# sparsemat/sprs

Hardware: AMD Instinct MI355X
Metric: CSR SpMV GFLOP/s (higher is better)
Workload: dtype f64; 1 GPU; R-MAT 10M x 10M, ~32 nnz/row (Graph500 a,b,c,d=.57,.19,.19,.05; seed 1); rows=10000000, cols=10000000, nnz=321592231, index_bytes=8, indptr_bytes=8, partition=single GPU, first_spmv_plan=nnz tiles

## Files before the change

sprs_amd/csrc/common.hpp:

```cpp
#pragma once

#include <hip/hip_runtime.h>
#include <cstdint>
#include <cstdio>
#include <memory>
#include <mutex>
#include <string>
#include <unordered_map>
#include <vector>

#include "../../include/sprs_hip.h"

struct sprs_hip_spgemm_plan;
struct sprs_hip_dist;

namespace sprs_hip {

void set_error(int32_t status, const char *fmt, ...) __attribute__((format(printf, 2, 3)));
int32_t fail_hip(hipError_t e, const char *what);
void clear_error();

#define SPRS_TRY_HIP(expr)                                              \
    do {                                                                \
        hipError_t e__ = (expr);                                        \
// ... 20 lines not shown
#define SPRS_HIP_OPTIONS(X)                                                                                                     \
    X(spmv_kernel, 0, 0, 2, 0)                                               \
    X(spmv_xcs, 0, 0, 2, 0)                                         \
    X(spmv_xcs_split, 32, 2, INT64_MAX, 0)                              \
    X(spmv_xcs_idx32, 1, 0, 1, 0)                                 \
    X(spmv_sort_tiles, 0, 0, 1, 0)               \
    X(spmv_relabel, 0, 0, 2, 0)                      \
    X(spmv_tile, 0, 0, 4096, 0)                                                 \
    X(spmv_lds_pad, 0, 0, 100000, 0)                  \
    X(spmv_xmask, -1, INT64_MIN, INT64_MAX, 1)       \
    X(spmv_plan_defer, 1, 0, 1, 0)       \
    X(spmv_band, 0, 0, 2, 0)                      \
    X(spmv_band_hot, 0, 0, 384, 0)                                                              \
    X(spmv_band_tile, 0, 0, 16384, 0)    \
    X(spmv_f32_band_tile, 0, 0, 32768, 0)  \
    X(spmv_band_phases, 0, 0, 8, 0)                        \
    X(spmv_band_split, 0, 0, INT64_MAX, 0)         \
    X(spmv_band_rounds, 0, 0, 64, 0)     \
    X(spmv_band_debug, 0, 0, 255, 1)     \
    X(spmv_band_tail, 0, 0, 2, 0)        \
    X(spmv_band_balance, 0, 0, 2, 0)     \
    X(spmv_band_xcd, 0, 0, 2, 0)         \
    X(spmv_band_pack, 0, 0, 2, 0)        \
    X(spmv_band_share, 0, 0, 1ll << 30, 0)  \
    X(spmv_band_hot_run, 0, 0, 4096, 0)  \
    X(spmv_band_cold_tiles, 0, 0, 64, 0)                  \
    X(spmv_band_overlap, 0, 0, 2, 0)         \
    X(spmv_band_split_permute, 0, 0, 2, 0)  \
    X(spmm_long_row, -1, -1, INT64_MAX, 0)  \
    X(spmm_stream, 1, 0, 1, 0)           \
    X(spgemm_micro, 0, 0, 2, 0)          \
    X(spgemm_task_order, 0, 0, 2, 0)      \
    X(spgemm_xcd_chunk, 0, -1, 0, 0)                \
    X(spgemm_bucket, 1, 0, 1, 0)                                   \
    X(spgemm_prof, 0, 0, 1, 1)                             \
    X(spgemm_tokens, 1, 1, 4, 0)                              \
    X(spgemm_keep_bits, 1, 0, 1, 0)      \
    X(spgemm_lane_order, 0, 0, 2, 0)     \
    X(spgemm_overlap, 0, 0, 1, 0)                                \
    X(spgemm_midwin_sym, 14, 14, 16, 0)                         \
    X(spgemm_mid_keep, 8, 4, 8, 0)       \
    X(spgemm_mid_keep_sym, 8, 8, 16, 0)  \
    X(spgemm_midwin, 15, 14, 15, 0)      \
    X(spgemm_mid, 65536, 0, 1ll << 31, 0)    \
    X(spgemm_ordered, 1, 0, 1, 0)        \
    X(spmm_relayout, 0, 0, 2, 0)         \
// ... 531 lines not shown
```

sprs_amd/csrc/spmv_band.hip:

```cpp
#include "spmv_band_kernels.hpp"

#include <algorithm>
#include <cstdlib>
#include <vector>

namespace sprs_hip {

namespace {

constexpr int MAX_HOT = 384;
constexpr int MAX_PHASES = 8;
constexpr int MAX_PIECES = MAX_HOT + 8 * MAX_PHASES + 1;

__global__ __launch_bounds__(256) void bp_inverse_kernel(const uint32_t *__restrict__ perm, uint64_t cols, uint32_t hot_labels,
                                                         uint32_t *__restrict__ inv_hot) {
    const uint64_t j = (uint64_t)blockIdx.x * blockDim.x + threadIdx.x;
    if (j >= cols) return;
    const uint32_t l = perm[j];
    if (l < hot_labels) inv_hot[l] = (uint32_t)j;
}

struct SliceMap {
    uint32_t nh, phases, xt_log2;
    uint64_t hot_labels;
    uint64_t phase_width;
};

__device__ __forceinline__ uint32_t piece_of_label(const SliceMap &m, uint64_t label) {
    if (label < m.hot_labels) return (uint32_t)(label >> m.xt_log2);
    uint64_t ph = (label - m.hot_labels) / m.phase_width;
    if (ph >= m.phases) ph = m.phases - 1;
    return m.nh + (uint32_t)ph * 8u + x_slice(label);
}

template <typename PTR>
__global__ void bp_classify_kernel(const PTR *__restrict__ indptr, uint64_t rows, uint64_t split,
                                   uint64_t *__restrict__ short_flag, uint64_t *__restrict__ short_len,
                                   uint64_t *__restrict__ long_flag) {
    const uint64_t r = (uint64_t)blockIdx.x * blockDim.x + threadIdx.x;
    if (r >= rows) return;
    const uint64_t len = (uint64_t)indptr[r + 1] - (uint64_t)indptr[r];
    const bool is_long = len >= split;
    short_flag[r] = (!is_long && len) ? 1 : 0;
    short_len[r] = is_long ? 0 : len;
    long_flag[r] = is_long ? 1 : 0;
}

struct ShortBuckets {
    const uint64_t *bucket0;
    uint64_t Rp, R;
};

__device__ __forceinline__ uint64_t short_place(const ShortBuckets &sb, uint64_t d) {
    if (!sb.bucket0) return d;
    const uint64_t k = d / sb.Rp;
    return k * sb.R + (d - sb.bucket0[k]);
}

__global__ void bp_bucket_starts_kernel(const uint64_t *__restrict__ short_ptr, uint64_t rows, uint64_t Rp, uint64_t nb,
                                        uint64_t *__restrict__ bucket0) {
    const uint64_t k = (uint64_t)blockIdx.x * blockDim.x + threadIdx.x;
    if (k >= nb) return;
    const uint64_t target = k * Rp;
    uint64_t lo = 0, hi = rows;
    while (lo < hi) {
        const uint64_t mid = (lo + hi) >> 1;
        if (short_ptr[mid] < target) lo = mid + 1;
        else hi = mid;
// ... 339 lines not shown
        if (fork) (void)hipEventDestroy(fork);
        if (join) (void)hipEventDestroy(join);
        if (aux) (void)hipStreamDestroy(aux);
    }
};

struct BandPlan {
    uint32_t nh = 0, phases = 1, npieces = 0;
    uint32_t xt_log2 = 14;
    uint32_t vbytes = 8;
    uint32_t n_long = 0, n_short_rows = 0;
    uint64_t cols = 0, cols_pad = 0;
    uint32_t *perm = nullptr, *long_rows = nullptr;
    uint32_t *inv_hot = nullptr;
    uint32_t nref = 0;
    uint32_t hot_labels = 0;
    void *vals_hot = nullptr, *vals_cold = nullptr;
    uint16_t *cid_hot = nullptr;
    unsigned char *packed_hot = nullptr;
    TileWord *hot_tw = nullptr;
    uint32_t hot_wgs_packed = 0;
    uint32_t *cid_cold = nullptr;
    uint32_t *rowidx_all = nullptr, *tile_row_all = nullptr;
    Seg *segs = nullptr;
    HotSeg *hsegs = nullptr;
    HotSeg *wg_first = nullptr;
    uint32_t *wg_seg = nullptr;
    uint32_t nranges = 0, nsegs = 0, hot_wgs = 0, cold_tiles = 4, hot_run = 4;
    void *spills_y = nullptr;
    void *rspills = nullptr;
    uint32_t *rsp_off = nullptr;
    uint32_t nspills = 0, nspills_y = 0;
    bool small = false;
    ColdGroup *groups = nullptr;
    unsigned long long *wmask = nullptr;
    uint32_t *wbase = nullptr;
    uint32_t np_pad = 0;
    uint64_t total_pairs = 0;
    uint32_t ngroups = 0, cold_blocks = 0, short_first_block = 0;
    bool has_short_group = false;
    std::vector<BandPiece> host_pieces;
    std::vector<uint64_t> pair_off;
    std::unordered_map<void *, BandScratch> scratch;
    uint64_t bytes = 0;
    DevBuf perm_block;
    std::vector<DevBuf> blocks;
// ... 197 lines not shown

    const uint64_t hot_entries = hot_tiles * WT;
    DevBuf vals_hot_blk, cid_hot_blk;
    SPRS_TRY_HIP(vals_hot_blk.alloc((hot_entries + WT) * VB));
    SPRS_TRY_HIP(cid_hot_blk.alloc((hot_entries + WT) * 2));
    bp->vals_hot = vals_hot_blk.p;
    bp->cid_hot = cid_hot_blk.as<uint16_t>();
    SPRS_TRY_HIP(hipMemsetAsync(bp->vals_hot, 0, (hot_entries + WT) * VB, stream));
    SPRS_TRY_HIP(hipMemsetAsync(bp->cid_hot, 0, (hot_entries + WT) * 2, stream));
    SPRS_TRY_HIP(alloc_block(bp->blocks, bp->vals_cold, (cold_ent + WT) * VB));
    SPRS_TRY_HIP(alloc_block(bp->blocks, bp->cid_cold, (cold_ent + WT) * 4));
    SPRS_TRY_HIP(hipMemsetAsync(bp->vals_cold, 0, (cold_ent + WT) * VB, stream));
    SPRS_TRY_HIP(hipMemsetD32Async((hipDeviceptr_t)bp->cid_cold, (int)(uint32_t)cols, cold_ent + WT, stream));
    DevBuf ptr_all;
    SPRS_TRY_HIP(ptr_all.alloc((ptr_off + n_short_rows + 2) * 4));
    SPRS_TRY_HIP(alloc_block(bp->blocks, bp->rowidx_all, (row_off + n_short_rows + 1) * 4));
    SPRS_TRY_HIP(alloc_block(bp->blocks, bp->tile_row_all, (tile_off + 1) * 4));
    bp->bytes = (cold_ent + WT) * (4 + VB) + (row_off + n_short_rows + tile_off) * 4 + cols * 4 + n_long * 4 +
                ((uint64_t)bp->nref + 4) * 4;
    hipLaunchKernelGGL((bp_fill_short_kernel<IDX, PTR, T>), dim3((unsigned)((rows + 256) / 256)), dim3(256), 0, stream, ip, ix,
                       (const T *)a->data, rows, short_pos.u64(), short_ptr.u64(), long_pos.u64(), bp->perm, (uint32_t *)nullptr,
                       (uint32_t *)s_ptr_t.p, bp->cid_cold, (T *)bp->vals_cold, bp->long_rows, split, 1, sbk, nnz_short_padded, n_long);
    SPRS_TRY_HIP(hipGetLastError());
    SPRS_TRY_HIP(hipMemcpyAsync((uint32_t *)ptr_all.p + ptr_off, s_ptr_t.p, (n_short_rows + 1) * 4, hipMemcpyDeviceToDevice, stream));
    if (n_short_rows)
        SPRS_TRY_HIP(hipMemcpyAsync(bp->rowidx_all + row_off, s_rowidx_t.p, n_short_rows * 4, hipMemcpyDeviceToDevice, stream));

    SPRS_TRY_HIP(pb_d.alloc(NP * sizeof(PieceBuild)));
    SPRS_TRY_HIP(hipMemcpyAsync(pb_d.p, pb.data(), NP * sizeof(PieceBuild), hipMemcpyHostToDevice, stream));
    hipLaunchKernelGGL((bp_scatter_kernel<IDX, PTR, T>), dim3((unsigned)wblocks), dim3(256), 0, stream, ip, ix, (const T *)a->data,
                       bp->long_rows, n_long, bp->perm, map, NP, pos.u64(), (const PieceBuild *)pb_d.p, (T *)bp->vals_hot,
                       bp->cid_hot, (T *)bp->vals_cold, bp->cid_cold);
    SPRS_TRY_HIP(hipGetLastError());
    hipLaunchKernelGGL(bp_rows_kernel, dim3((unsigned)((flat + 255) / 256)), dim3(256), 0, stream, cnt.u64(), pos.u64(),
                       pair.u64(), n_long, NP, (const PieceBuild *)pb_d.p, (uint32_t *)ptr_all.p, bp->rowidx_all);
    SPRS_TRY_HIP(hipGetLastError());

    {
        const uint64_t nwb = (n_long + WAVE - 1) / WAVE;
        bp->total_pairs = row_off;
        bp->np_pad = (NP + (uint32_t)RU - 1u) / (uint32_t)RU * (uint32_t)RU;
        const uint64_t slots = nwb * bp->np_pad;
        SPRS_TRY_HIP(alloc_block(bp->blocks, bp->wmask, (slots + WAVE) * 8));
        SPRS_TRY_HIP(alloc_block(bp->blocks, bp->wbase, (slots + WAVE) * 4));
        SPRS_TRY_HIP(hipMemsetAsync(bp->wmask, 0, (slots + WAVE) * 8, stream));
        SPRS_TRY_HIP(hipMemsetAsync(bp->wbase, 0, (slots + WAVE) * 4, stream));
// ... 318 lines not shown
    return dispatch_widths(a->idx_bytes, a->iptr_bytes, [&](auto i, auto p) {
        return band_build_t<typename decltype(i)::type, typename decltype(p)::type>(a, stream, out);
    });
}

int32_t band_prepare_stream(sprs_hip_csmat_f32 *a, BandPlan *bp, hipStream_t stream) {
    std::lock_guard<std::recursive_mutex> lock(a->mu);
    BandScratch *sc = nullptr;
    return band_scratch(bp, stream, &sc);
}

uint64_t band_plan_bytes(const BandPlan *bp) { return bp ? bp->bytes : 0; }

namespace {
template <typename T>
struct BandK;
template <>
struct BandK<double> {
    using Cold = ColdArgs;
    using Reduce = ReduceArgs;
    template <bool ACC, bool TOY>
    static auto cold() { return &band_cold_kernel<ACC, TOY>; }
    template <bool ACC>
    static auto reduce() { return &band_reduce_kernel<ACC>; }
    template <bool ACC>
    static auto tail() { return &band_tail_kernel<ACC>; }
    static auto permute() { return &band_permute_kernel; }
};
template <>
struct BandK<float> {
    using Cold = ColdArgsT<float>;
    using Reduce = ReduceArgsT<float>;
    template <bool ACC, bool TOY>
    static auto cold() { return &band_cold_kernel_f32<ACC, TOY>; }
    template <bool ACC>
    static auto reduce() { return &band_reduce_kernel_f32<ACC>; }
    template <bool ACC>
    static auto tail() { return &band_tail_kernel_f32<ACC>; }
    static auto permute() { return &band_permute_kernel_f32; }
};

template <typename H>
int32_t band_spmv_t(H *a, BandPlan *bp, const typename H::value_type *x, typename H::value_type *y, bool acc, hipStream_t stream) {
    using T = typename H::value_type;
    using K = BandK<T>;
    constexpr bool F32 = sizeof(T) == 4;
    BandScratch *sc = nullptr;
    {
        std::lock_guard<std::recursive_mutex> lock(a->mu);
        SPRS_TRY(band_scratch(bp, stream, &sc));
    }
    const bool overlap = options().spmv_band_overlap != 2 && bp->hot_wgs && bp->cold_blocks && (!bp->small || options().spmv_band_overlap == 1);
    const bool split_permute = overlap && options().spmv_band_split_permute != 2 && bp->hot_labels;
    const bool early_reduce = overlap && options().spmv_band_tail != 2;
    hipStream_t cstream = overlap ? sc->aux : stream;
    auto launch_carry_y = [&](hipStream_t st) -> int32_t {
        const uint32_t n = bp->nspills_y;
        if (!n) return SPRS_HIP_OK;
        hipLaunchKernelGGL((band_carry_kernel<true, T>), dim3((n + 255) / 256), dim3(256), 0, st, (const Spill *)bp->spills_y, n, (const T *)sc->carry,
                           (T *)sc->partial, y);
        SPRS_TRY_HIP(hipGetLastError());
        return SPRS_HIP_OK;
    };
    const uint32_t cut = bp->has_short_group ? bp->short_first_block : bp->cold_blocks;
    const bool fused_tail = !overlap && bp->small && options().spmv_band_tail != 2 && bp->cold_blocks > cut;
    auto launch_hot = [&]() -> int32_t {
        if (!bp->hot_wgs) return SPRS_HIP_OK;
        const uint32_t lds = F32 ? hot_lds_bytes_f32(bp->xt_log2) : hot_lds_bytes(bp->xt_log2);
#ifndef SPRS_HIP_EMU
        {
            static std::mutex mu;
            static std::unordered_map<int, bool> done;
            std::lock_guard<std::mutex> lock(mu);
            if constexpr (F32) {
                if (!done[a->device]) {
                    SPRS_TRY_HIP(hipFuncSetAttribute((const void *)band_hot_kernel_f32<13, 0>, hipFuncAttributeMaxDynamicSharedMemorySize, (int)hot_lds_bytes_f32(13)));
                    SPRS_TRY_HIP(hipFuncSetAttribute((const void *)band_hot_kernel_f32<14, 0>, hipFuncAttributeMaxDynamicSharedMemorySize, (int)hot_lds_bytes_f32(14)));
                    SPRS_TRY_HIP(hipFuncSetAttribute((const void *)band_hot_kernel_f32<15, 0>, hipFuncAttributeMaxDynamicSharedMemorySize, (int)hot_lds_bytes_f32(15)));
                    done[a->device] = true;
                }
            } else if (!done[a->device]) {
                const void *k13[] = {(const void *)band_hot_kernel<13, 0>, (const void *)band_hot_kernel<13, 1>, (const void *)band_hot_kernel<13, 2>};
                const void *k14[] = {(const void *)band_hot_kernel<14, 0>, (const void *)band_hot_kernel<14, 1>, (const void *)band_hot_kernel<14, 2>};
                for (const void *k : k13) SPRS_TRY_HIP(hipFuncSetAttribute(k, hipFuncAttributeMaxDynamicSharedMemorySize, (int)hot_lds_bytes(13)));
                for (const void *k : k14) SPRS_TRY_HIP(hipFuncSetAttribute(k, hipFuncAttributeMaxDynamicSharedMemorySize, (int)hot_lds_bytes(14)));
                done[a->device] = true;
            }
        }
// ... 49 lines not shown
                t1 = std::max(t1, t[3 * b + 2]);
            }
            std::vector<double> st, xw, du, en;
            for (uint32_t b = 0; b < bp->hot_wgs; ++b) {
                st.push_back((t[3 * b] - t0) * 0.01);
                xw.push_back((t[3 * b + 1] - t[3 * b]) * 0.01);
                du.push_back((t[3 * b + 2] - t[3 * b]) * 0.01);
                en.push_back((t[3 * b + 2] - t0) * 0.01);
            }
            auto q = [](std::vector<double> v, double f) {
                std::sort(v.begin(), v.end());
                return v[(size_t)(f * (v.size() - 1))];
            };
            fprintf(stderr, "[hot_prof] %u workgroups, span %.1f us | start min/med/p90/max %.1f %.1f %.1f %.1f | first x tile after %.1f %.1f %.1f %.1f | "
                            "duration %.1f %.1f %.1f %.1f | end %.1f %.1f %.1f %.1f\n", bp->hot_wgs, (t1 - t0) * 0.01,
                    q(st, 0), q(st, .5), q(st, .9), q(st, 1), q(xw, 0), q(xw, .5), q(xw, .9), q(xw, 1), q(du, 0), q(du, .5), q(du, .9), q(du, 1),
                    q(en, 0), q(en, .5), q(en, .9), q(en, 1));
        }
        return SPRS_HIP_OK;
    };
    auto cold_args = [&](uint32_t b0) {
        typename K::Cold ca;
        static_cast<ColdArgsT<T> &>(ca) = ColdArgsT<T>{sc->pieces, bp->groups, bp->ngroups, (const T *)bp->vals_cold, bp->cid_cold, (const T *)sc->xp, y, (T *)sc->carry,
                                                       b0, bp->cold_tiles, 0u, BandPiece()};
        return ca;
    };
    auto launch_gather = [&](uint32_t b0, uint32_t nb) -> int32_t {
        if (!nb) return SPRS_HIP_OK;
        const typename K::Cold ca = cold_args(b0);
        if (b0 < cut) hipLaunchKernelGGL((K::template cold<false, false>()), dim3(nb), dim3(CNT), 0, cstream, ca);
        else if (acc) hipLaunchKernelGGL((K::template cold<true, true>()), dim3(nb), dim3(CNT), 0, cstream, ca);
        else hipLaunchKernelGGL((K::template cold<false, true>()), dim3(nb), dim3(CNT), 0, cstream, ca);
        SPRS_TRY_HIP(hipGetLastError());
        return SPRS_HIP_OK;
    };

    const bool by_gather = (uint64_t)bp->nref * 3 <= bp->cols;
    auto launch_xp = [&](uint32_t l0, uint32_t l1, bool clear_y, hipStream_t st, bool hot_only = false) -> int32_t {
        if (!by_gather && !hot_only) {
            const uint64_t span = clear_y ? std::max<uint64_t>(bp->cols, a->rows) : bp->cols;
            hipLaunchKernelGGL((K::permute()), dim3((unsigned)((span + 1023) / 1024)), dim3(256), 0, st, x, (const uint32_t *)bp->perm, bp->cols,
                               (T *)sc->xp, clear_y ? y : (T *)nullptr, a->rows, l0, (uint32_t)bp->cols_pad);
            SPRS_TRY_HIP(hipGetLastError());
            return SPRS_HIP_OK;
        }
        const uint64_t n4 = std::max<uint64_t>(l1 > l0 ? ((uint64_t)(l1 - l0) + 3) / 4 : 0, clear_y ? (a->rows + 3) / 4 : 0);
        if (!n4) return SPRS_HIP_OK;
        if (clear_y)
            hipLaunchKernelGGL((band_gather_kernel<true, T>), dim3((unsigned)((n4 + 255) / 256)), dim3(256), 0, st, x, (const uint32_t *)bp->inv_hot, l0,
                               l1 > l0 ? l1 : l0, (T *)sc->xp, y, a->rows);
        else
            hipLaunchKernelGGL((band_gather_kernel<false, T>), dim3((unsigned)((n4 + 255) / 256)), dim3(256), 0, st, x, (const uint32_t *)bp->inv_hot, l0,
                               l1 > l0 ? l1 : l0, (T *)sc->xp, (T *)nullptr, a->rows);
        SPRS_TRY_HIP(hipGetLastError());
        return SPRS_HIP_OK;
    };
    const uint32_t hot_end = bp->hot_labels < bp->nref ? bp->hot_labels : bp->nref;
    if (split_permute) SPRS_TRY(launch_xp(0u, hot_end, false, stream, true));
    else SPRS_TRY(launch_xp(0u, bp->nref, !acc, stream));
    if (overlap) {
        SPRS_TRY_HIP(hipEventRecord(sc->fork, stream));
        SPRS_TRY(launch_hot());
        SPRS_TRY_HIP(hipStreamWaitEvent(sc->aux, sc->fork, 0));
    }
    if (split_permute) SPRS_TRY(launch_xp(hot_end, bp->nref, !acc, cstream));
    SPRS_TRY(launch_gather(0, cut));
    if (early_reduce) SPRS_TRY_HIP(hipEventRecord(sc->cold_done, sc->aux));
    if (!fused_tail) SPRS_TRY(launch_gather(cut, bp->cold_blocks - cut));
    if (early_reduce) SPRS_TRY(launch_carry_y(sc->aux));
    if (overlap) SPRS_TRY_HIP(hipEventRecord(sc->join, sc->aux));
    else SPRS_TRY(launch_hot());
    if (overlap) SPRS_TRY_HIP(hipStreamWaitEvent(stream, early_reduce ? sc->cold_done : sc->join, 0));
    if (!early_reduce && !fused_tail) SPRS_TRY(launch_carry_y(stream));
    const uint32_t nwb = (bp->n_long + WAVE - 1) / WAVE;
    const uint32_t per_xcd = (nwb + 7) / 8;
    const dim3 rg(((per_xcd + 3) / 4) * 8), rb(256);
    typename K::Reduce ra;
    static_cast<ReduceArgsT<T> &>(ra) = ReduceArgsT<T>{(const T *)sc->partial, bp->wmask, bp->wbase, bp->long_rows, (const RSpill *)bp->rspills,
                                                       bp->nspills ? bp->rsp_off : nullptr, (const T *)sc->carry, y, bp->n_long, bp->np_pad, nwb};
    if (fused_tail) {
        typename K::Cold ca = cold_args(cut);
        ca.direct = 1u;
        ca.piece = bp->host_pieces[bp->npieces];
        const dim3 tg(rg.x + (bp->cold_blocks - cut));
        if (acc) hipLaunchKernelGGL((K::template tail<true>()), tg, rb, 0, stream, ra, rg.x, ca);
        else hipLaunchKernelGGL((K::template tail<false>()), tg, rb, 0, stream, ra, rg.x, ca);
        SPRS_TRY_HIP(hipGetLastError());
        SPRS_TRY(launch_carry_y(stream));
    } else {
        if (acc) hipLaunchKernelGGL((K::template reduce<true>()), rg, rb, 0, stream, ra);
        else hipLaunchKernelGGL((K::template reduce<false>()), rg, rb, 0, stream, ra);
        SPRS_TRY_HIP(hipGetLastError());
    }
    if (early_reduce) SPRS_TRY_HIP(hipStreamWaitEvent(stream, sc->join, 0));
    return SPRS_HIP_OK;
}
}

int32_t band_spmv(sprs_hip_csmat *a, BandPlan *bp, const double *x, double *y, bool acc, hipStream_t stream) {
    return band_spmv_t(a, bp, x, y, acc, stream);
}
int32_t band_spmv(sprs_hip_csmat_f32 *a, BandPlan *bp, const float *x, float *y, bool acc, hipStream_t stream) {
    return band_spmv_t(a, bp, x, y, acc, stream);
}

}
```

sprs_amd/csrc/spmv_band_kernels.hpp:

```cpp
#pragma once
#include "spmv_shared.hpp"

namespace sprs_hip {
namespace {

typedef uint32_t u32x4 __attribute__((ext_vector_type(4)));
typedef float flt4 __attribute__((ext_vector_type(4)));

constexpr int WT = 512;
constexpr int WPASS = WT / (WAVE * 2);
constexpr int EPL = WT / WAVE;
constexpr int HOT_THREADS = 1024;
constexpr int HOT_WAVES = HOT_THREADS / WAVE;
constexpr int CNT = 256;
constexpr uint32_t ROW_START = 0x8000u;
constexpr uint32_t KEY_SEL = 0x4000u;
constexpr uint32_t ROW_START32 = 0x80000000u;
static_assert(WPASS == 4 && EPL == 8, "wave tile geometry");

template <typename T>
struct BandT;
template <>
struct BandT<double> {
    typedef dbl2 vec;
// ... 125 lines not shown
__device__ __forceinline__ float band_lane_below(float S, uint32_t lane) {
    (void)lane;
    return __builtin_bit_cast(float, __builtin_amdgcn_update_dpp(0, __builtin_bit_cast(int, S), 0x138, 0xf, 0xf, true));
}

__device__ __forceinline__ double band_read_lane63(double v) {
    const int lo = __builtin_amdgcn_readlane(__double2loint(v), WAVE - 1);
    const int hi = __builtin_amdgcn_readlane(__double2hiint(v), WAVE - 1);
    return __hiloint2double(hi, lo);
}
__device__ __forceinline__ float band_read_lane63(float v) {
    return __builtin_bit_cast(float, __builtin_amdgcn_readlane(__builtin_bit_cast(int, v), WAVE - 1));
}

__device__ __forceinline__ double band_read_lane(double v, int src) {
    const int lo = __builtin_amdgcn_readlane(__double2loint(v), src);
    const int hi = __builtin_amdgcn_readlane(__double2hiint(v), src);
    return __hiloint2double(hi, lo);
}
__device__ __forceinline__ float band_read_lane(float v, int src) {
    return __builtin_bit_cast(float, __builtin_amdgcn_readlane(__builtin_bit_cast(int, v), src));
}

__device__ __forceinline__ void wave_lds_fence() {
    __builtin_amdgcn_fence(__ATOMIC_RELEASE, "wavefront");
    __builtin_amdgcn_wave_barrier();
    __builtin_amdgcn_fence(__ATOMIC_ACQUIRE, "wavefront");
}

constexpr int STG = 128;
constexpr uint32_t hot_lds_bytes(uint32_t xt_log2) { return ((1u << xt_log2) + (uint32_t)HOT_WAVES * 128u) * 8u; }
constexpr uint32_t hot_lds_bytes_f32(uint32_t xt_log2) { return ((1u << xt_log2) + (uint32_t)HOT_WAVES * 128u) * 4u; }

struct Pending {
    uint32_t cnt = 0;
    uint32_t row0 = 0;
    bool first_to_carry = false;
};

template <typename T, typename Out>
__device__ __forceinline__ void band_flush(Pending &pd, uint32_t lane, SPRS_GLOBAL_AS T *carry, const T *stage, Out out) {
    for (uint32_t j = lane; j < pd.cnt; j += WAVE) {
        const T v = stage[j];
        if (j == 0 && pd.first_to_carry) *carry = v;
        else out(pd.row0 + j, v);
    }
    wave_lds_fence();
    pd.cnt = 0;
}

template <bool DEFER, typename T, typename Out>
__device__ __forceinline__ void band_tile_sums(const T (&pr)[EPL], uint32_t fb, uint32_t lane, uint32_t R0, T &open, bool &mine,
                                               uint32_t &last, SPRS_GLOBAL_AS T *carry, T *stage, Pending &pd, Out out) {
    const uint32_t nfl = (uint32_t)__popc(fb);
    const uint32_t incl = band_scan_incl_u32(nfl, lane);
    const uint32_t prefix = incl - nfl;
    const uint32_t nf = (uint32_t)__builtin_amdgcn_readlane((int)incl, WAVE - 1);
    T ev[EPL];
    T run = 0.0, head = 0.0;
    uint32_t seen = 0;
#pragma unroll
    for (int q = 0; q < EPL; ++q) {
        ev[q] = run;
        if ((fb >> q) & 1u) {
// ... 12 lines not shown
    for (uint32_t lo = 0; lo < nf; lo += STG) {
#pragma unroll
        for (int q = 0; q < EPL; ++q) {
            if ((fb >> q) & 1u) {
                const uint32_t below = fb & ((1u << q) - 1u);
                const uint32_t o = prefix + (uint32_t)__popc(below) - lo;
                if (o < (uint32_t)STG) stage[o] = below ? ev[q] : vhead;
            }
        }
        wave_lds_fence();
        pd.cnt = nf - lo < (uint32_t)STG ? nf - lo : (uint32_t)STG;
        pd.row0 = R0 - 1u + lo;
        pd.first_to_carry = lo == 0 && !mine;
        if (!DEFER || lo + STG < nf) band_flush(pd, lane, carry, stage, out);
    }
    const T s63 = band_read_lane63(S);
    open = nf ? s63 : open + s63;
    if (nf) {
        mine = true;
        last = R0 + nf - 1;
    }
}

template <bool ACC, bool TOY, typename T>
__device__ __forceinline__ void band_cold_wave(const PieceView<T> d, uint32_t r, uint32_t ct, const T *__restrict__ vals,
                                               const uint32_t *__restrict__ cid, const T *__restrict__ xp, T *__restrict__ y,
                                               T *__restrict__ carry, T *stage, uint32_t lane);

template <typename T>
struct ColdArgsT {
    const BandPiece *pieces;
    const ColdGroup *groups;
    uint32_t ngroups;
    const T *vals;
    const uint32_t *cid;
    const T *xp;
    T *y, *carry;
    uint32_t block0, ct;
    uint32_t direct;
    BandPiece piece;
};
struct ColdArgs : ColdArgsT<double> {};

template <bool ACC, bool TOY, typename T>
__device__ __forceinline__ void band_cold_body(const ColdArgsT<T> &ca, uint32_t block, T (*stage_s)[STG]) {
    constexpr int WPB = CNT / WAVE;
    const BandPiece *__restrict__ pieces = ca.pieces;
    const ColdGroup *__restrict__ groups = ca.groups;
    const uint32_t ngroups = ca.ngroups, ct = ca.ct;
    const T *__restrict__ vals = ca.vals;
    const uint32_t *__restrict__ cid = ca.cid;
    const T *__restrict__ xp = ca.xp;
    T *__restrict__ y = ca.y;
    T *__restrict__ carry = ca.carry;
    const uint32_t tid = threadIdx.x, lane = tid & (WAVE - 1), wave = tid / WAVE;
    T *stage = stage_s[wave];
    const uint32_t bid = block + ca.block0;
    uint32_t r;
    BandPiece pc;
    if (ca.direct) {
        pc = ca.piece;
        r = block * WPB + wave;
    } else {
        uint32_t g = 0;
        while (g + 1 < ngroups && bid >= groups[g + 1].first_block) ++g;
        const ColdGroup cg = groups[g];
        const uint32_t lb = bid - cg.first_block;
        const uint32_t pi = cg.first_piece + (cg.npieces == 1 ? 0u : (lb & 7u));
        r = (cg.npieces == 1 ? lb : (lb >> 3)) * WPB + wave;
        pc = pieces[pi];
    }
    band_cold_wave<ACC, TOY, T>(PieceView<T>(pc), r, ct, vals, cid, xp, y, carry, stage, lane);
}

template <bool ACC, bool TOY, typename T>
__device__ __forceinline__ void band_cold_wave(const PieceView<T> d, uint32_t r, uint32_t ct, const T *__restrict__ vals,
                                               const uint32_t *__restrict__ cid, const T *__restrict__ xp, T *__restrict__ y,
                                               T *__restrict__ carry, T *stage, uint32_t lane) {
    typedef typename BandT<T>::vec vecT;
    constexpr int VW = BandT<T>::VW, NV = BandT<T>::NV;
    const uint32_t t0 = r * ct;
    if (t0 >= d.ntiles) return;
    const uint32_t tend = t0 + ct < d.ntiles ? t0 + ct : d.ntiles;
    vecT av[NV];
    u32x4 lw[2];
    uint32_t R0n = 0;
    auto request = [&](uint32_t w) {
        const uint64_t gpos = d.ent0 + (uint64_t)w * WT;
#pragma unroll
        for (int p = 0; p < 2; ++p) lw[p] = __builtin_nontemporal_load((const u32x4 *)(cid + gpos + p * (WAVE * 4) + lane * 4));
#pragma unroll
        for (int p = 0; p < NV; ++p) av[p] = __builtin_nontemporal_load((const vecT *)(vals + gpos + p * (WAVE * VW) + lane * VW));
        R0n = d.tile_row[w];
    };
    request(t0);
    T open = 0.0;
    bool mine = false;
    uint32_t last = 0;
    SPRS_GLOBAL_AS T *cslot = (SPRS_GLOBAL_AS T *)carry + d.range0 + r;
    uint32_t yr_pre[4] = {0u, 0u, 0u, 0u}, yr_base = 0;
    auto emit_y = [&](uint32_t row, T v) {
        const uint32_t m = (row - yr_base) >> 6;
        uint32_t yr;
        if (TOY && m < 4u && ((row - yr_base) & 63u) == lane) yr = m == 0 ? yr_pre[0] : m == 1 ? yr_pre[1] : m == 2 ? yr_pre[2] : yr_pre[3];
        else yr = d.rowidx[row];
        if constexpr (ACC) y[yr] = y[yr] + v;
        else y[yr] = v;
    };
    auto emit_p = [&](uint32_t row, T v) { d.out[row] = v; };
    for (uint32_t w = t0; w < tend; ++w) {
        const uint64_t base = (uint64_t)w * WT;
        const uint32_t cnt = d.nnz - base < (uint64_t)WT ? (uint32_t)(d.nnz - base) : (uint32_t)WT;
        T xv[EPL];
        uint32_t fb = 0;
#pragma unroll
        for (int q = 0; q < EPL; ++q) {
            const uint32_t c = lw[q / 4][q % 4];
            xv[q] = xp[c & ~ROW_START32];
            fb |= (c >> 31) << q;
        }
        if constexpr (TOY) {
            yr_base = R0n - 1u;
#pragma unroll
            for (int m = 0; m < 4; ++m) {
                const uint32_t rr = yr_base + lane + 64u * (uint32_t)m;
                yr_pre[m] = d.rowidx[rr < d.nr ? rr : d.nr - 1u];
            }
        }
        T pr[EPL];
#pragma unroll
        for (int q = 0; q < EPL; ++q) pr[q] = av[q / VW][q % VW] * xv[q];
        if (cnt < (uint32_t)WT) {
#pragma unroll
            for (int q = 0; q < EPL; ++q) pr[q] = lane * EPL + q < cnt ? pr[q] : (T)0.0;
        }
        Pending pd;
        if constexpr (TOY) band_tile_sums<false>(pr, fb, lane, R0n, open, mine, last, cslot, stage, pd, emit_y);
        else band_tile_sums<false>(pr, fb, lane, R0n, open, mine, last, cslot, stage, pd, emit_p);
        if (w + 1 < tend) request(w + 1);
    }
    if (lane == 0) {
        if (!mine) *cslot = open;
        else if constexpr (TOY) emit_y(last, open);
        else emit_p(last, open);
    }
}

template <bool ACC, bool TOY>
__global__ __launch_bounds__(CNT, 8) void band_cold_kernel(ColdArgs ca) {
    __shared__ __attribute__((aligned(16))) double stage_s[CNT / WAVE][STG];
    band_cold_body<ACC, TOY, double>(ca, blockIdx.x, stage_s);
}
template <bool ACC, bool TOY>
__global__ __launch_bounds__(CNT, 8) void band_cold_kernel_f32(ColdArgsT<float> ca) {
    __shared__ __attribute__((aligned(16))) float stage_s[CNT / WAVE][STG];
    band_cold_body<ACC, TOY, float>(ca, blockIdx.x, stage_s);
}

struct RangeRef {
    uint32_t piece, tile0;
    bool valid;
};

__device__ __forceinline__ RangeRef range_of(const Seg *__restrict__ segs, uint32_t nsegs, uint32_t i) {
    uint32_t lo = 0, hi = nsegs;
    while (hi - lo > 1) {
        const uint32_t mid = (lo + hi) >> 1;
        if (segs[mid].range0 <= i) lo = mid;
        else hi = mid;
    }
    const Seg sg = segs[lo];
    const uint32_t t = (i - sg.range0) * sg.run;
    return RangeRef{sg.piece, sg.tile0 + t, t < sg.ntiles};
}

__device__ __forceinline__ bool range_has_head(const BandPiece &d, uint32_t piece, uint32_t tile0, const uint16_t *__restrict__ cid_hot,
                                               const uint32_t *__restrict__ cid_cold, uint32_t nhot) {
    const uint64_t e = d.ent0 + (uint64_t)tile0 * WT;
    return piece < nhot ? !(cid_hot[e] & ROW_START) : !(cid_cold[e] & ROW_START32);
// ... 59 lines not shown
template <bool CLEAR_Y, typename T>
__global__ __launch_bounds__(256) void band_gather_kernel(const T *__restrict__ x, const uint32_t *__restrict__ inv, uint32_t l0,
                                                          uint32_t l1, T *__restrict__ xp, T *__restrict__ y_zero, uint64_t rows) {
    const uint64_t t4 = ((uint64_t)blockIdx.x * blockDim.x + threadIdx.x) * 4;
    const uint64_t l = (uint64_t)l0 + t4;
    if (l + 4 <= (uint64_t)l1 && (l0 & 3u) == 0) {
        const u32x4 j = *(const u32x4 *)(inv + l);
        const T a0 = x[j[0]], a1 = x[j[1]], a2 = x[j[2]], a3 = x[j[3]];
        band_store4(xp + l, a0, a1, a2, a3);
    } else {
        for (uint64_t q = l; q < (uint64_t)l1 && q < l + 4; ++q) xp[q] = x[inv[q]];
    }
    if (CLEAR_Y && y_zero) {
        if (t4 + 4 <= rows && ((uintptr_t)y_zero & 15) == 0) {
            band_store4(y_zero + t4, (T)0.0, (T)0.0, (T)0.0, (T)0.0);
        } else {
            for (uint64_t r = t4; r < rows && r < t4 + 4; ++r) y_zero[r] = 0.0;
        }
    }
}


constexpr int RU = 16;

__device__ __forceinline__ bool band_mask_bit(uint32_t m_lo, uint32_t m_hi, uint32_t lane) {
    (void)lane;
    return __builtin_amdgcn_inverse_ballot_w64(((unsigned long long)m_hi << 32) | m_lo);
}
__device__ __forceinline__ uint32_t band_mask_rank(uint32_t m_lo, uint32_t m_hi, uint32_t lane) {
    (void)lane;
    return __builtin_amdgcn_mbcnt_hi(m_hi, __builtin_amdgcn_mbcnt_lo(m_lo, 0u));
}

template <typename T>
struct ReduceArgsT {
    const T *partial;
    const unsigned long long *wmask;
    const uint32_t *wbase, *long_rows;
    const RSpill *rsp;
    const uint32_t *rsp_off;
    const T *carry;
    T *y;
    uint32_t n_long, np_pad, nwb;
};
struct ReduceArgs : ReduceArgsT<double> {};

template <bool ACC, typename T>
__device__ __forceinline__ void band_reduce_body(const ReduceArgsT<T> &ra, uint32_t block, uint32_t nblocks) {
    const T *__restrict__ partial = ra.partial;
    const unsigned long long *__restrict__ wmask = ra.wmask;
    const uint32_t *__restrict__ wbase = ra.wbase;
    const uint32_t *__restrict__ long_rows = ra.long_rows;
    T *__restrict__ y = ra.y;
    const uint32_t n_long = ra.n_long, np_pad = ra.np_pad, nwb = ra.nwb;
    const uint32_t lane = threadIdx.x & (WAVE - 1);
// ... 70 lines not shown
                if (lane == tj) s += hv;
            }
        }
        if (j < n_long) {
            if constexpr (ACC) y[r] = y[r] + s;
            else y[r] = s;
        }
    }
}

template <bool ACC>
__global__ __launch_bounds__(256) void band_reduce_kernel(ReduceArgs ra) {
    band_reduce_body<ACC, double>(ra, blockIdx.x, gridDim.x);
}
template <bool ACC>
__global__ __launch_bounds__(256) void band_reduce_kernel_f32(ReduceArgsT<float> ra) {
    band_reduce_body<ACC, float>(ra, blockIdx.x, gridDim.x);
}

template <bool ACC>
__global__ __launch_bounds__(CNT, 8) void band_tail_kernel(ReduceArgs ra, uint32_t reduce_blocks, ColdArgs ca) {
    __shared__ __attribute__((aligned(16))) double stage_s[CNT / WAVE][STG];
    if (blockIdx.x < reduce_blocks) band_reduce_body<ACC, double>(ra, blockIdx.x, reduce_blocks);
    else band_cold_body<ACC, true, double>(ca, blockIdx.x - reduce_blocks, stage_s);
}
template <bool ACC>
__global__ __launch_bounds__(CNT, 8) void band_tail_kernel_f32(ReduceArgsT<float> ra, uint32_t reduce_blocks, ColdArgsT<float> ca) {
    __shared__ __attribute__((aligned(16))) float stage_s[CNT / WAVE][STG];
    if (blockIdx.x < reduce_blocks) band_reduce_body<ACC, float>(ra, blockIdx.x, reduce_blocks);
    else band_cold_body<ACC, true, float>(ca, blockIdx.x - reduce_blocks, stage_s);
}

#define BAND_T double
#define BAND_KERNEL(name) name
#include "spmv_band_twins.inc"
#undef BAND_T
#undef BAND_KERNEL
#define BAND_T float
#define BAND_KERNEL(name) name##_f32
#include "spmv_band_twins.inc"
#undef BAND_T
#undef BAND_KERNEL

}
}
```

Baseline: 629.7 GFLOP/s.

## Write y once from short-row band kernel, skipping separate y zeroing

Adds per-wave bitmasks of short and long rows, built at plan time. The short-row cold kernel then writes every non-long y entry in row windows, storing zeros for empty rows. This lets the gather/permute step skip its pass that clears y, saving a full write of y (10M doubles) per SpMV. In exchange, the flush gets mask lookups, ballot and rank logic, and extra window bookkeeping, all added to the cold kernel's inner path.

```diff
diff --git a/sprs_amd/csrc/common.hpp b/sprs_amd/csrc/common.hpp
--- a/sprs_amd/csrc/common.hpp
+++ b/sprs_amd/csrc/common.hpp
@@ -66,6 +66,7 @@
     X(spmv_band_balance, 0, 0, 2, 0)     \
     X(spmv_band_xcd, 0, 0, 2, 0)         \
     X(spmv_band_pack, 0, 0, 2, 0)        \
+    X(spmv_band_y_once, 0, 0, 2, 0)      \
     X(spmv_band_share, 0, 0, 1ll << 30, 0)  \
     X(spmv_band_hot_run, 0, 0, 4096, 0)  \
     X(spmv_band_cold_tiles, 0, 0, 64, 0)                  \
diff --git a/sprs_amd/csrc/spmv_band.hip b/sprs_amd/csrc/spmv_band.hip
--- a/sprs_amd/csrc/spmv_band.hip
+++ b/sprs_amd/csrc/spmv_band.hip
@@ -44,6 +44,18 @@
     short_flag[r] = (!is_long && len) ? 1 : 0;
     short_len[r] = is_long ? 0 : len;
     long_flag[r] = is_long ? 1 : 0;
+}
+
+template <typename PTR>
+__global__ __launch_bounds__(256) void bp_row_masks_kernel(const PTR *__restrict__ indptr, uint64_t rows, uint64_t split,
+                                                           unsigned long long *__restrict__ is_short, unsigned long long *__restrict__ is_long) {
+    const uint64_t r = (uint64_t)blockIdx.x * blockDim.x + threadIdx.x;
+    const uint64_t len = r < rows ? (uint64_t)indptr[r + 1] - (uint64_t)indptr[r] : 0;
+    const unsigned long long ms = __ballot(len != 0 && len < split), ml = __ballot(len >= split);
+    if ((threadIdx.x & (WAVE - 1)) == 0 && r < rows) {
+        is_short[r / WAVE] = ms;
+        is_long[r / WAVE] = ml;
+    }
 }
 
 struct ShortBuckets {
@@ -429,6 +441,8 @@
     uint32_t hot_wgs_packed = 0;
     uint32_t *cid_cold = nullptr;
     uint32_t *rowidx_all = nullptr, *tile_row_all = nullptr;
+    unsigned long long *is_short = nullptr, *is_long = nullptr;
+    uint64_t rows = 0;
     Seg *segs = nullptr;
     HotSeg *hsegs = nullptr;
     HotSeg *wg_first = nullptr;
@@ -672,6 +686,15 @@
                        (const T *)a->data, rows, short_pos.u64(), short_ptr.u64(), long_pos.u64(), bp->perm, (uint32_t *)nullptr,
                        (uint32_t *)s_ptr_t.p, bp->cid_cold, (T *)bp->vals_cold, bp->long_rows, split, 1, sbk, nnz_short_padded, n_long);
     SPRS_TRY_HIP(hipGetLastError());
+    bp->rows = rows;
+    if (n_short_rows) {
+        const uint64_t words = (rows + WAVE - 1) / WAVE;
+        SPRS_TRY_HIP(alloc_block(bp->blocks, bp->is_short, (words + 1) * 8));
+        SPRS_TRY_HIP(alloc_block(bp->blocks, bp->is_long, (words + 1) * 8));
+        hipLaunchKernelGGL(bp_row_masks_kernel<PTR>, dim3((unsigned)((words + 3) / 4)), dim3(256), 0, stream, ip, rows, split, bp->is_short, bp->is_long);
+        SPRS_TRY_HIP(hipGetLastError());
+        bp->bytes += words * 16;
+    }
     SPRS_TRY_HIP(hipMemcpyAsync((uint32_t *)ptr_all.p + ptr_off, s_ptr_t.p, (n_short_rows + 1) * 4, hipMemcpyDeviceToDevice, stream));
     if (n_short_rows)
         SPRS_TRY_HIP(hipMemcpyAsync(bp->rowidx_all + row_off, s_rowidx_t.p, n_short_rows * 4, hipMemcpyDeviceToDevice, stream));
@@ -1036,6 +1059,10 @@
     template <bool ACC, bool TOY>
     static auto cold() { return &band_cold_kernel<ACC, TOY>; }
     template <bool ACC>
+    static auto short_once() { return &band_short_kernel<ACC>; }
+    template <bool ACC>
+    static auto tail_once() { return &band_tail_once_kernel<ACC>; }
+    template <bool ACC>
     static auto reduce() { return &band_reduce_kernel<ACC>; }
     template <bool ACC>
     static auto tail() { return &band_tail_kernel<ACC>; }
@@ -1047,6 +1074,10 @@
     using Reduce = ReduceArgsT<float>;
     template <bool ACC, bool TOY>
     static auto cold() { return &band_cold_kernel_f32<ACC, TOY>; }
+    template <bool ACC>
+    static auto short_once() { return &band_short_kernel_f32<ACC>; }
+    template <bool ACC>
+    static auto tail_once() { return &band_tail_once_kernel_f32<ACC>; }
     template <bool ACC>
     static auto reduce() { return &band_reduce_kernel_f32<ACC>; }
     template <bool ACC>
@@ -1078,6 +1109,7 @@
     };
     const uint32_t cut = bp->has_short_group ? bp->short_first_block : bp->cold_blocks;
     const bool fused_tail = !overlap && bp->small && options().spmv_band_tail != 2 && bp->cold_blocks > cut;
+    const bool y_once = options().spmv_band_y_once != 2 && bp->is_short && bp->cold_blocks > cut;
     auto launch_hot = [&]() -> int32_t {
         if (!bp->hot_wgs) return SPRS_HIP_OK;
         const uint32_t lds = F32 ? hot_lds_bytes_f32(bp->xt_log2) : hot_lds_bytes(bp->xt_log2);
@@ -1173,13 +1205,17 @@
     auto cold_args = [&](uint32_t b0) {
         typename K::Cold ca;
         static_cast<ColdArgsT<T> &>(ca) = ColdArgsT<T>{sc->pieces, bp->groups, bp->ngroups, (const T *)bp->vals_cold, bp->cid_cold, (const T *)sc->xp, y, (T *)sc->carry,
-                                                       b0, bp->cold_tiles, 0u, BandPiece()};
+                                                       b0, bp->cold_tiles, 0u, BandPiece(),
+                                                       YOnce{y_once ? bp->is_short : nullptr, y_once ? bp->is_long : nullptr, (uint32_t)bp->rows,
+                                                             DEVTOOLS ? (uint32_t)options().spmv_band_debug : 0u}};
         return ca;
     };
     auto launch_gather = [&](uint32_t b0, uint32_t nb) -> int32_t {
         if (!nb) return SPRS_HIP_OK;
         const typename K::Cold ca = cold_args(b0);
         if (b0 < cut) hipLaunchKernelGGL((K::template cold<false, false>()), dim3(nb), dim3(CNT), 0, cstream, ca);
+        else if (y_once && acc) hipLaunchKernelGGL((K::template short_once<true>()), dim3(nb), dim3(CNT), 0, cstream, ca);
+        else if (y_once) hipLaunchKernelGGL((K::template short_once<false>()), dim3(nb), dim3(CNT), 0, cstream, ca);
         else if (acc) hipLaunchKernelGGL((K::template cold<true, true>()), dim3(nb), dim3(CNT), 0, cstream, ca);
         else hipLaunchKernelGGL((K::template cold<false, true>()), dim3(nb), dim3(CNT), 0, cstream, ca);
         SPRS_TRY_HIP(hipGetLastError());
@@ -1188,18 +1224,19 @@
 
     const bool by_gather = (uint64_t)bp->nref * 3 <= bp->cols;
     auto launch_xp = [&](uint32_t l0, uint32_t l1, bool clear_y, hipStream_t st, bool hot_only = false) -> int32_t {
+        const bool zero_y = clear_y && !y_once;
         if (!by_gather && !hot_only) {
-            const uint64_t span = clear_y ? std::max<uint64_t>(bp->cols, a->rows) : bp->cols;
+            const uint64_t span = zero_y ? std::max<uint64_t>(bp->cols, a->rows) : bp->cols;
             hipLaunchKernelGGL((K::permute()), dim3((unsigned)((span + 1023) / 1024)), dim3(256), 0, st, x, (const uint32_t *)bp->perm, bp->cols,
-                               (T *)sc->xp, clear_y ? y : (T *)nullptr, a->rows, l0, (uint32_t)bp->cols_pad);
+                               (T *)sc->xp, zero_y ? y : (T *)nullptr, a->rows, l0, (uint32_t)bp->cols_pad);
             SPRS_TRY_HIP(hipGetLastError());
             return SPRS_HIP_OK;
         }
-        const uint64_t n4 = std::max<uint64_t>(l1 > l0 ? ((uint64_t)(l1 - l0) + 3) / 4 : 0, clear_y ? (a->rows + 3) / 4 : 0);
+        const uint64_t n4 = std::max<uint64_t>(l1 > l0 ? ((uint64_t)(l1 - l0) + 3) / 4 : 0, zero_y ? (a->rows + 3) / 4 : 0);
         if (!n4) return SPRS_HIP_OK;
         if (clear_y)
             hipLaunchKernelGGL((band_gather_kernel<true, T>), dim3((unsigned)((n4 + 255) / 256)), dim3(256), 0, st, x, (const uint32_t *)bp->inv_hot, l0,
-                               l1 > l0 ? l1 : l0, (T *)sc->xp, y, a->rows);
+                               l1 > l0 ? l1 : l0, (T *)sc->xp, zero_y ? y : (T *)nullptr, a->rows);
         else
             hipLaunchKernelGGL((band_gather_kernel<false, T>), dim3((unsigned)((n4 + 255) / 256)), dim3(256), 0, st, x, (const uint32_t *)bp->inv_hot, l0,
                                l1 > l0 ? l1 : l0, (T *)sc->xp, (T *)nullptr, a->rows);
@@ -1234,7 +1271,9 @@
         ca.direct = 1u;
         ca.piece = bp->host_pieces[bp->npieces];
         const dim3 tg(rg.x + (bp->cold_blocks - cut));
-        if (acc) hipLaunchKernelGGL((K::template tail<true>()), tg, rb, 0, stream, ra, rg.x, ca);
+        if (y_once && acc) hipLaunchKernelGGL((K::template tail_once<true>()), tg, rb, 0, stream, ra, rg.x, ca);
+        else if (y_once) hipLaunchKernelGGL((K::template tail_once<false>()), tg, rb, 0, stream, ra, rg.x, ca);
+        else if (acc) hipLaunchKernelGGL((K::template tail<true>()), tg, rb, 0, stream, ra, rg.x, ca);
         else hipLaunchKernelGGL((K::template tail<false>()), tg, rb, 0, stream, ra, rg.x, ca);
         SPRS_TRY_HIP(hipGetLastError());
         SPRS_TRY(launch_carry_y(stream));
diff --git a/sprs_amd/csrc/spmv_band_kernels.hpp b/sprs_amd/csrc/spmv_band_kernels.hpp
--- a/sprs_amd/csrc/spmv_band_kernels.hpp
+++ b/sprs_amd/csrc/spmv_band_kernels.hpp
@@ -171,6 +171,15 @@
     return __builtin_bit_cast(float, __builtin_amdgcn_readlane(__builtin_bit_cast(int, v), src));
 }
 
+__device__ __forceinline__ bool band_mask_bit(uint32_t m_lo, uint32_t m_hi, uint32_t lane) {
+    (void)lane;
+    return __builtin_amdgcn_inverse_ballot_w64(((unsigned long long)m_hi << 32) | m_lo);
+}
+__device__ __forceinline__ uint32_t band_mask_rank(uint32_t m_lo, uint32_t m_hi, uint32_t lane) {
+    (void)lane;
+    return __builtin_amdgcn_mbcnt_hi(m_hi, __builtin_amdgcn_mbcnt_lo(m_lo, 0u));
+}
+
 __device__ __forceinline__ void wave_lds_fence() {
     __builtin_amdgcn_fence(__ATOMIC_RELEASE, "wavefront");
     __builtin_amdgcn_wave_barrier();
@@ -187,8 +196,29 @@
     bool first_to_carry = false;
 };
 
+template <typename Emit, typename Window>
+struct BandWindowOut {
+    Emit emit;
+    Window window;
+    bool whole;
+    template <typename T>
+    __device__ __forceinline__ void operator()(uint32_t row, T v) const { emit(row, v); }
+};
+template <typename Out>
+struct band_takes_windows { static constexpr bool value = false; };
+template <typename Emit, typename Window>
+struct band_takes_windows<BandWindowOut<Emit, Window>> { static constexpr bool value = true; };
+
 template <typename T, typename Out>
 __device__ __forceinline__ void band_flush(Pending &pd, uint32_t lane, SPRS_GLOBAL_AS T *carry, const T *stage, Out out) {
+    if constexpr (band_takes_windows<Out>::value) {
+        if (out.whole) {
+            out.window(pd, carry);
+            wave_lds_fence();
+            pd.cnt = 0;
+            return;
+        }
+    }
     for (uint32_t j = lane; j < pd.cnt; j += WAVE) {
         const T v = stage[j];
         if (j == 0 && pd.first_to_carry) *carry = v;
@@ -247,10 +277,15 @@
     }
 }
 
-template <bool ACC, bool TOY, typename T>
+struct YOnce {
+    const unsigned long long *is_short, *is_long;
+    uint32_t rows, dbg;
+};
+
+template <bool ACC, bool TOY, bool YONCE, typename T>
 __device__ __forceinline__ void band_cold_wave(const PieceView<T> d, uint32_t r, uint32_t ct, const T *__restrict__ vals,
                                                const uint32_t *__restrict__ cid, const T *__restrict__ xp, T *__restrict__ y,
-                                               T *__restrict__ carry, T *stage, uint32_t lane);
+                                               T *__restrict__ carry, T *stage, uint32_t lane, const YOnce yo);
 
 template <typename T>
 struct ColdArgsT {
@@ -264,10 +299,11 @@
     uint32_t block0, ct;
     uint32_t direct;
     BandPiece piece;
+    YOnce yo;
 };
 struct ColdArgs : ColdArgsT<double> {};
 
-template <bool ACC, bool TOY, typename T>
+template <bool ACC, bool TOY, bool YONCE, typename T>
 __device__ __forceinline__ void band_cold_body(const ColdArgsT<T> &ca, uint32_t block, T (*stage_s)[STG]) {
     constexpr int WPB = CNT / WAVE;
     const BandPiece *__restrict__ pieces = ca.pieces;
@@ -295,18 +331,20 @@
         r = (cg.npieces == 1 ? lb : (lb >> 3)) * WPB + wave;
         pc = pieces[pi];
     }
-    band_cold_wave<ACC, TOY, T>(PieceView<T>(pc), r, ct, vals, cid, xp, y, carry, stage, lane);
-}
-
-template <bool ACC, bool TOY, typename T>
+    band_cold_wave<ACC, TOY, YONCE, T>(PieceView<T>(pc), r, ct, vals, cid, xp, y, carry, stage, lane, ca.yo);
+}
+
+template <bool ACC, bool TOY, bool YONCE, typename T>
 __device__ __forceinline__ void band_cold_wave(const PieceView<T> d, uint32_t r, uint32_t ct, const T *__restrict__ vals,
                                                const uint32_t *__restrict__ cid, const T *__restrict__ xp, T *__restrict__ y,
-                                               T *__restrict__ carry, T *stage, uint32_t lane) {
+                                               T *__restrict__ carry, T *stage, uint32_t lane, const YOnce yo) {
     typedef typename BandT<T>::vec vecT;
     constexpr int VW = BandT<T>::VW, NV = BandT<T>::NV;
     const uint32_t t0 = r * ct;
     if (t0 >= d.ntiles) return;
     const uint32_t tend = t0 + ct < d.ntiles ? t0 + ct : d.ntiles;
+    static_assert(TOY || !YONCE, "only the short rows write y");
+    constexpr bool y_once = YONCE;
     vecT av[NV];
     u32x4 lw[2];
     uint32_t R0n = 0;
@@ -318,7 +356,10 @@
         for (int p = 0; p < NV; ++p) av[p] = __builtin_nontemporal_load((const vecT *)(vals + gpos + p * (WAVE * VW) + lane * VW));
         R0n = d.tile_row[w];
     };
+    uint32_t ycur = 0, rf = 0;
+    if (y_once && r) rf = d.tile_row[t0];
     request(t0);
+    if (y_once && r) ycur = d.rowidx[rf < d.nr ? rf : d.nr - 1u];
     T open = 0.0;
     bool mine = false;
     uint32_t last = 0;
@@ -333,6 +374,43 @@
         else y[yr] = v;
     };
     auto emit_p = [&](uint32_t row, T v) { d.out[row] = v; };
+    auto window_y = [&](const Pending &p, SPRS_GLOBAL_AS T *cs) {
+        uint32_t base = 0;
+        if (p.first_to_carry) {
+            if (lane == 0) *cs = stage[0];
+            base = 1;
+        }
+        uint32_t yc = (uint32_t)__builtin_amdgcn_readfirstlane((int)ycur);
+        while (yc < yo.rows) {
+            const uint32_t wd = yc >> 6, b0 = yc & 63u;
+            unsigned long long ms = yo.is_short[wd] & (~0ull << b0);
+            const unsigned long long ml = yo.is_long[wd];
+            const uint32_t avail = p.cnt - base;
+            uint32_t end = WAVE;
+            if ((uint32_t)__popcll(ms) > avail) {
+                const bool at = ((ms >> lane) & 1ull) && band_mask_rank((uint32_t)ms, (uint32_t)(ms >> 32), lane) == avail;
+                end = (uint32_t)__builtin_ctzll(__ballot(at));
+                ms &= (1ull << end) - 1ull;
+            }
+            const bool sh = (ms >> lane) & 1ull;
+            const uint32_t row = (wd << 6) + lane;
+            if (lane >= b0 && lane < end && row < yo.rows && !((ml >> lane) & 1ull) && !(DEVTOOLS && (yo.dbg & 32u))) {
+                if constexpr (ACC) {
+                    if (sh) y[row] = y[row] + stage[base + band_mask_rank((uint32_t)ms, (uint32_t)(ms >> 32), lane)];
+                } else {
+                    y[row] = sh ? stage[base + band_mask_rank((uint32_t)ms, (uint32_t)(ms >> 32), lane)] : (T)0.0;
+                }
+            }
+            base += (uint32_t)__popcll(ms);
+            if (end < (uint32_t)WAVE) {
+                yc = (wd << 6) + end;
+                break;
+            }
+            yc = ((uint64_t)wd + 1u) * WAVE < (uint64_t)yo.rows ? (wd + 1u) << 6 : yo.rows;
+        }
+        ycur = yc;
+    };
+    BandWindowOut<decltype(emit_y), decltype(window_y)> out_y{emit_y, window_y, y_once};
     for (uint32_t w = t0; w < tend; ++w) {
         const uint64_t base = (uint64_t)w * WT;
         const uint32_t cnt = d.nnz - base < (uint64_t)WT ? (uint32_t)(d.nnz - base) : (uint32_t)WT;
@@ -344,7 +422,7 @@
             xv[q] = xp[c & ~ROW_START32];
             fb |= (c >> 31) << q;
         }
-        if constexpr (TOY) {
+        if (TOY && !y_once) {
             yr_base = R0n - 1u;
 #pragma unroll
             for (int m = 0; m < 4; ++m) {
@@ -360,11 +438,18 @@
             for (int q = 0; q < EPL; ++q) pr[q] = lane * EPL + q < cnt ? pr[q] : (T)0.0;
         }
         Pending pd;
-        if constexpr (TOY) band_tile_sums<false>(pr, fb, lane, R0n, open, mine, last, cslot, stage, pd, emit_y);
+        if constexpr (TOY) band_tile_sums<false>(pr, fb, lane, R0n, open, mine, last, cslot, stage, pd, out_y);
         else band_tile_sums<false>(pr, fb, lane, R0n, open, mine, last, cslot, stage, pd, emit_p);
         if (w + 1 < tend) request(w + 1);
     }
-    if (lane == 0) {
+    if (y_once && mine) {
+        if (lane == 0) stage[0] = open;
+        wave_lds_fence();
+        Pending pl;
+        pl.cnt = 1;
+        pl.row0 = last;
+        window_y(pl, cslot);
+    } else if (lane == 0) {
         if (!mine) *cslot = open;
         else if constexpr (TOY) emit_y(last, open);
         else emit_p(last, open);
@@ -374,12 +459,22 @@
 template <bool ACC, bool TOY>
 __global__ __launch_bounds__(CNT, 8) void band_cold_kernel(ColdArgs ca) {
     __shared__ __attribute__((aligned(16))) double stage_s[CNT / WAVE][STG];
-    band_cold_body<ACC, TOY, double>(ca, blockIdx.x, stage_s);
+    band_cold_body<ACC, TOY, false, double>(ca, blockIdx.x, stage_s);
 }
 template <bool ACC, bool TOY>
 __global__ __launch_bounds__(CNT, 8) void band_cold_kernel_f32(ColdArgsT<float> ca) {
     __shared__ __attribute__((aligned(16))) float stage_s[CNT / WAVE][STG];
-    band_cold_body<ACC, TOY, float>(ca, blockIdx.x, stage_s);
+    band_cold_body<ACC, TOY, false, float>(ca, blockIdx.x, stage_s);
+}
+template <bool ACC>
+__global__ __launch_bounds__(CNT, 8) void band_short_kernel(ColdArgs ca) {
+    __shared__ __attribute__((aligned(16))) double stage_s[CNT / WAVE][STG];
+    band_cold_body<ACC, true, true, double>(ca, blockIdx.x, stage_s);
+}
+template <bool ACC>
+__global__ __launch_bounds__(CNT, 8) void band_short_kernel_f32(ColdArgsT<float> ca) {
+    __shared__ __attribute__((aligned(16))) float stage_s[CNT / WAVE][STG];
+    band_cold_body<ACC, true, true, float>(ca, blockIdx.x, stage_s);
 }
 
 struct RangeRef {
@@ -485,15 +580,6 @@
 
 
 constexpr int RU = 16;
-
-__device__ __forceinline__ bool band_mask_bit(uint32_t m_lo, uint32_t m_hi, uint32_t lane) {
-    (void)lane;
-    return __builtin_amdgcn_inverse_ballot_w64(((unsigned long long)m_hi << 32) | m_lo);
-}
-__device__ __forceinline__ uint32_t band_mask_rank(uint32_t m_lo, uint32_t m_hi, uint32_t lane) {
-    (void)lane;
-    return __builtin_amdgcn_mbcnt_hi(m_hi, __builtin_amdgcn_mbcnt_lo(m_lo, 0u));
-}
 
 template <typename T>
 struct ReduceArgsT {
@@ -610,13 +696,26 @@
 __global__ __launch_bounds__(CNT, 8) void band_tail_kernel(ReduceArgs ra, uint32_t reduce_blocks, ColdArgs ca) {
     __shared__ __attribute__((aligned(16))) double stage_s[CNT / WAVE][STG];
     if (blockIdx.x < reduce_blocks) band_reduce_body<ACC, double>(ra, blockIdx.x, reduce_blocks);
-    else band_cold_body<ACC, true, double>(ca, blockIdx.x - reduce_blocks, stage_s);
+    else band_cold_body<ACC, true, false, double>(ca, blockIdx.x - reduce_blocks, stage_s);
 }
 template <bool ACC>
 __global__ __launch_bounds__(CNT, 8) void band_tail_kernel_f32(ReduceArgsT<float> ra, uint32_t reduce_blocks, ColdArgsT<float> ca) {
     __shared__ __attribute__((aligned(16))) float stage_s[CNT / WAVE][STG];
     if (blockIdx.x < reduce_blocks) band_reduce_body<ACC, float>(ra, blockIdx.x, reduce_blocks);
-    else band_cold_body<ACC, true, float>(ca, blockIdx.x - reduce_blocks, stage_s);
+    else band_cold_body<ACC, true, false, float>(ca, blockIdx.x - reduce_blocks, stage_s);
+}
+
+template <bool ACC>
+__global__ __launch_bounds__(CNT, 8) void band_tail_once_kernel(ReduceArgs ra, uint32_t reduce_blocks, ColdArgs ca) {
+    __shared__ __attribute__((aligned(16))) double stage_s[CNT / WAVE][STG];
+    if (blockIdx.x < reduce_blocks) band_reduce_body<ACC, double>(ra, blockIdx.x, reduce_blocks);
+    else band_cold_body<ACC, true, true, double>(ca, blockIdx.x - reduce_blocks, stage_s);
+}
+template <bool ACC>
+__global__ __launch_bounds__(CNT, 8) void band_tail_once_kernel_f32(ReduceArgsT<float> ra, uint32_t reduce_blocks, ColdArgsT<float> ca) {
+    __shared__ __attribute__((aligned(16))) float stage_s[CNT / WAVE][STG];
+    if (blockIdx.x < reduce_blocks) band_reduce_body<ACC, float>(ra, blockIdx.x, reduce_blocks);
+    else band_cold_body<ACC, true, true, float>(ca, blockIdx.x - reduce_blocks, stage_s);
 }
 
 #define BAND_T double
```

Measured after the change: 566.0 GFLOP/s. 0.899x the previous value.
